# facebookresearch/holo_diffusion

Measured on AMD Instinct MI355X. Metric: denoise-steps/sec + rendered-rays/sec, 64^3x32 grid @400^2 render, higher is better.
Workload: dtype f32

## Files before the change

### holo_diffusion_amd/csrc/holo_knobs.h

```cpp
#pragma once

#include <stdint.h>
#include <stdlib.h>

namespace holo {

#ifdef HOLO_EMU
constexpr bool EMU_BUILD = true;
#else
constexpr bool EMU_BUILD = false;
#endif

constexpr int64_t KNOB_UNSET = INT64_MIN;

#define HOLO_KNOBS(X)                                                                                                      \
  X(num_cus, "HOLO_NUM_CUS", POS, 0, CTX, "planners size grids and split-K for this many CUs (default: the device's)")     \
  X(conv_wino, "HOLO_CONV_WINO", INT, 1, HANDLE, "0: no Winograd copies of the conv weights (forward and dgrad)")          \
  X(conv_wino3, "HOLO_CONV_WINO3", INT, 1, HANDLE_PLAN, "0: no F(2x2x2, 3x3x3) copies / conv_wino3_kernel never chosen")   \
  X(keep_intermediates, "HOLO_KEEP_INTERMEDIATES", CH, '1', HANDLE,                                                        \
    "1: the plan releases no activation, holo_unet_fetch_block works")                                                     \
  X(render_v1, "HOLO_RENDER_V1", SET, 0, HANDLE, "the ray-per-column render kernel for everything")                        \
  X(render2_nw, "HOLO_RENDER2_NW", INT, 0, HANDLE, "8: the 8-wave form of render2_kernel's 12-wave configurations")        \
  X(render2_nrm_nw, "HOLO_RENDER2_NRM_NW", INT, 0, HANDLE,                                                                 \
    "8: rendered normals two waves per SIMD instead of 10 waves (the emulation build always runs 8)")                      \
  X(render_wgs, "HOLO_RENDER_WGS", POS, 0, HANDLE, "persistent render workgroups (default: one per CU)")                   \
  X(render_xcd, "HOLO_RENDER_XCD", RAW, KNOB_UNSET, HANDLE,                                                                \
    "XCD ranges of the render tile order (default 8; 2 in the emulation build; <= 1: plain order)")                        \
  X(render_tail, "HOLO_RENDER_TAIL", RAW, KNOB_UNSET, HANDLE,                                                              \
    "4-ray tiles at the end of every XCD range handed out as single rays (default: about two rounds; 3 in the "            \
    "emulation build; 0: off)")                                                                                            \
  X(render_static_tiles, "HOLO_RENDER_STATIC_TILES", SET, 0, HANDLE, "static tile stride instead of the dynamic hand-out") \
  X(render_timeline, "HOLO_RENDER_TIMELINE", SET, 0, HANDLE, "per-phase clocks of every render launch (synchronises!)")    \
  X(mlp_mean_bwd_chunk, "HOLO_MLP_MEAN_BWD_CHUNK", POS, 0, HANDLE,                                                         \
    "voxels per chunk of holo_mlp_mean_backward (default: what fits 4 GiB of rows; the emulation build: always 2048)")     \
  X(conv_wino_small, "HOLO_CONV_WINO_SMALL", INT, 1, PLAN, "0: under-filled levels take 64-voxel tiles, not Winograd")     \
  X(conv_force_tz2, "HOLO_CONV_FORCE_TZ2", INT, 0, PLAN, "1: 128-voxel tiles (hence the Winograd kernels) on small grids") \
  X(conv_qkv_fused, "HOLO_CONV_QKV_FUSED", INT, 1, PLAN, "0: row-tile qkv convolution + attn_pack_kernel")                 \
  X(conv1x1_bf16_stream, "HOLO_CONV1X1_BF16_STREAM", INT, 1, PLAN, "0: the row-tile kernel for bf16 1x1x1 convolutions")   \
  X(conv1x1_stream_min_m, "HOLO_CONV1X1_STREAM_MIN_M", INT, 131072, PLAN,                                                  \
    "rows from which a raw-input fp32 1x1x1 convolution streams (0: never)")                                               \
  X(conv1x1_small, "HOLO_CONV1X1_SMALL", INT, 1, PLAN, "0: the row-tile kernel for the fp32 attention's 1x1x1 convs")      \
  X(conv_s2t, "HOLO_CONV_S2T", INT, -1, PLAN, "stride-2 bf16 halo kernel: 0 never, 1 wherever defined (default: by fill)") \
  X(conv_bf16t, "HOLO_CONV_BF16T", INT, -1, PLAN, "bf16 wide-tile kernel: 0 never, 1 everywhere (default: by fill / K)")   \
  X(conv_bf16p, "HOLO_CONV_BF16P", INT, -1, PLAN,                                                                          \
    "its persistent form: 0 never, 1 every wide-tile launch, 2 activated input too (default: raw input)")                  \
  X(conv_bf16p_wgs, "HOLO_CONV_BF16P_WGS", INT, 0, PLAN, "at most this many persistent workgroups (0: no cap)")            \
  X(conv_wino3_min_items, "HOLO_CONV_WINO3_MIN_ITEMS", INT, KNOB_UNSET, PLAN,                                              \
    "work items from which conv_wino3_kernel runs (default: num_cus / 2)")                                                 \
  X(conv_wino3_up, "HOLO_CONV_WINO3_UP", INT, 1, PLAN,                                                                     \
    "0: upsampling convolutions on conv_wino3_kernel's generic form (64 pseudo-taps), not its 27-tap form")               \
  X(no_skip_fusion, "HOLO_NO_SKIP_FUSION", SET, 0, PLAN, "a ResBlock's 1x1x1 skip always as its own launch")               \
  X(skip_fusion_below_r, "HOLO_SKIP_FUSION_BELOW_R", RAW, 64, PLAN,                                                        \
    "exact fp32: the skip is fused into the second convolution below this grid edge")                                      \
  X(no_flash_attn, "HOLO_NO_FLASH_ATTN", SET, 0, PLAN, "attention as GEMM + softmax + GEMM")                               \
  X(bf16_flash_min_t, "HOLO_BF16_FLASH_MIN_T", RAW, 1024, PLAN, "tokens from which the bf16 mode takes its bf16 attention") \
  X(flash_split, "HOLO_FLASH_SPLIT", INT, 0, PLAN, "key splits of the fp32 attention, clamped to [1, T/128] (0: by fill)") \
  X(flash_v2_ksplit, "HOLO_FLASH_V2_KSPLIT", INT, 0, PLAN,                                                                 \
    "key splits of the bf16 attention: 1..8 dividing T into multiples of 128, else ignored")                               \
  X(attn_exact, "HOLO_ATTN_EXACT", SET, 0, PLAN, "bf16 attention: the exact loop alone, no LAZY pass")                     \
  X(debug_timestep_load, "HOLO_DEBUG_TIMESTEP_LOAD", INT, 0, PLAN, "how time_embed_kernel loads the timesteps (see it)")   \
  X(dgrad_s2_direct, "HOLO_DGRAD_S2_DIRECT", CH, '1', PLAN, "1: conv_dgrad_s2_kernel for every Downsample dgrad")          \
  X(wgrad_tiles, "HOLO_WGRAD_TILES", POS, 0, PLAN, "> 0: the tile weight-gradient kernel instead of the row-staged one")   \
  X(wgrad_reduce_tile_min, "HOLO_WGRAD_REDUCE_TILE_MIN", RAW, 1024, PLAN,                                                  \
    "64-element tiles from which the weight-gradient reduce runs its tile form")                                           \
  X(debug_plan, "HOLO_DEBUG_PLAN", SET, 0, PLAN, "[plan] lines on stderr: what every convolution / attention launches")    \
  X(viewpool_bwd_v1, "HOLO_VIEWPOOL_BWD_V1", CH, '1', CALL, "1: the register-accumulating view-pool backward kernel")      \
  HOLO_KNOBS_DEV(X)

#ifdef HOLO_DEV_PROBES
#define HOLO_KNOBS_DEV(X)                                                                                                  \
  X(viewpool_bwd_probe, "HOLO_VIEWPOOL_BWD_PROBE", RAW, KNOB_UNSET, CALL,                                                  \
    "view-pool backward: 0 no pass 2, 2 pass 2 without its atomics, 10 + k the atomics of map k alone")                    \
  X(viewpool_bwd_occ, "HOLO_VIEWPOOL_BWD_OCC", CH, '3', CALL, "view-pool backward: 3 = the 166-register build")
#else
#define HOLO_KNOBS_DEV(X)
#endif

typedef int64_t knob_INT_t, knob_RAW_t, knob_POS_t;
typedef bool knob_SET_t, knob_CH_t;
static inline int64_t knob_INT(const char* e, int64_t dflt) { return e && e[0] ? strtoll(e, nullptr, 10) : dflt; }
static inline int64_t knob_RAW(const char* e, int64_t dflt) { return e ? atoll(e) : dflt; }
static inline bool knob_SET(const char* e, int) { return e != nullptr; }
static inline bool knob_CH(const char* e, char c) { return e && e[0] == c; }
static inline int64_t knob_POS(const char* e, int) { return e && atoll(e) > 0 ? atoll(e) : 0; }

struct Knobs {
// ... 14 lines not shown
```

### holo_diffusion_amd/csrc/unet_exec.cpp

```cpp
#include <math.h>
#include <stdarg.h>
#include <stdio.h>
#include <stdlib.h>
#include <string.h>

#include <functional>
#include <map>
#include <optional>
#include <string>
#include <vector>

#include "../../include/holo_abi.h"
#include "conv_weights.h"
#include "holo_common.h"
#include "holo_kernels.h"

namespace holo {

static thread_local char g_err[512] = "";
void set_error(const char* fmt, ...) {
  va_list ap;
  va_start(ap, fmt);
  vsnprintf(g_err, sizeof(g_err), fmt, ap);
  va_end(ap);
}
const char* get_error() { return g_err; }

#define HIP_TRY(expr)                                                                  \
  do {                                                                                 \
    hipError_t _e = (expr);                                                            \
    if (_e != hipSuccess) {                                                            \
      set_error("%s failed: %s (%s:%d)", #expr, hipGetErrorString(_e), __FILE__, __LINE__); \
      return HOLO_E_HIP;                                                               \
    }                                                                                  \
  } while (0)

}

// ... 94 lines not shown
  Act x0, x1, h1, out;
  bool has_x1 = false;
  size_t coefA = 0, coefB = 0, momA = 0, momB = 0;
  const float* film = nullptr;
  size_t qkv = 0, a = 0;
  bool has_skip = false;
};

enum OpKind { OP_IN = 1, OP_TEMB, OP_EMBLIN, OP_STATS, OP_FINAL, OP_CONV, OP_GEMM, OP_SOFTMAX, OP_FLASH, OP_OUT };
struct LayoutIn { float* dst; int C; int64_t V; int dst_bf16; };
struct LayoutOut { const float* src; int C; int64_t V; };
struct TimeEmbed {
  const float *w1, *b1, *w2, *b2;
  float *emb, *emb_silu;
  int load_kind;
};
struct EmbLinears {
  const float *emb_silu, *w, *b;
  float* out;
};
struct GnStats {
  const float* x;
  double* part;
  int C, x_bf16;
  int64_t V;
};
struct GnFinalize {
  const double *part0, *part1;
  int C0, B0, C1, B1;
  int64_t V;
  const float *gamma, *beta, *film;
  int film_stride, film_cout;
  float *coef, *moments;
};
struct Softmax { float* S; int64_t rows; int cols; };
struct Flash {
  AttnParams attn;
  int form;
  float* packed;
  int out_bf16;
  int operands_packed;
  int ksplit, lazy;
};
struct Op {
  OpKind kind;
  union {
    LayoutIn in;
    TimeEmbed temb;
    EmbLinears emblin;
    GnStats stats;
    GnFinalize fin;
    ConvParams conv;
    GemmParams gemm;
    Softmax softmax;
    Flash flash;
    LayoutOut out;
  };
};
static Op make_op(OpKind kind) {
  Op op;
  memset(&op, 0, sizeof op);
  op.kind = kind;
  return op;
}

struct Plan {
  int batch = -1;
  void* ws = nullptr;
  std::vector<Op> ops;
  size_t bytes = 0;
  std::map<std::string, Act> block_outputs;
  int first_conv = -1, last_conv = -1;
  const char* cl_refusal = nullptr;
  bool built_for(int b, const void* w) const { return batch == b && ws == w && !ops.empty(); }
  void invalidate() { *this = Plan(); }
};
struct TrainPlan {
  Plan fwd;
  std::vector<std::function<int(void*)>> bops;
  std::vector<size_t> grad_off;
  size_t gy_off = 0, gx_off = 0;
  size_t bytes = 0;
  bool built_for(int b, const void* w) const { return fwd.built_for(b, w); }
  void invalidate() { *this = TrainPlan(); }
};

}

struct HoloUnet {
  HoloCtx* ctx;
  HoloUnetCfg cfg;
  std::vector<std::vector<Block>> inputs, outputs;
  std::vector<Block> middle;
  int final_ch;
  int ted;
  std::vector<ParamSlot> params;
  std::map<std::string, int> pindex;
  float* pstore = nullptr;
  uint16_t* pstore_bf = nullptr;
  float* pstore_wino = nullptr;
  int compute_mode = 0;
  bool batch_invariant = false;
  int emb_rows = 0;
  std::map<std::string, int> emb_row_off;
  float* emb_w = nullptr;
  float* emb_b = nullptr;
  Knobs knobs;
  Plan plan;
  std::map<std::pair<int, bool>, size_t> ws_cache;
  std::map<std::string, ConvWeights> dgrad;
  std::vector<float*> adam_copies;
  float* dgrad_tmp = nullptr;
  TrainPlan tplan;
  const int64_t* t_dev = nullptr;
  bool tape_valid = false;
  std::map<int, size_t> tws_cache;
};

namespace {

void build_structure(HoloUnet* u) {
  const HoloUnetCfg& c = u->cfg;
  const int mc = c.model_channels;
  int ch = c.channel_mult[0] * mc;
  char buf[128];
  u->inputs.clear();
  u->outputs.clear();
  u->middle.clear();
  u->inputs.push_back({Block{B_CONV, "input_blocks.0.0", c.in_channels, ch}});
  std::vector<int> chans{ch};
  int ds = 1, idx = 1;
  auto has_attn = [&](int d) {
    for (int i = 0; i < c.n_attention_resolutions; ++i)
      if (c.attention_resolutions[i] == d) return true;
    return false;
  };
  for (int level = 0; level < c.n_channel_mult; ++level) {
    const int mult = c.channel_mult[level];
    for (int r = 0; r < c.num_res_blocks; ++r) {
      std::vector<Block> layers;
      snprintf(buf, sizeof buf, "input_blocks.%d.0", idx);
      layers.push_back(Block{B_RES, buf, ch, mult * mc});
      ch = mult * mc;
      if (has_attn(ds)) {
        snprintf(buf, sizeof buf, "input_blocks.%d.1", idx);
        layers.push_back(Block{B_ATTN, buf, ch, ch});
      }
      u->inputs.push_back(layers);
      chans.push_back(ch);
// ... 149 lines not shown
    }
  return n;
}

ConvWeights W(const HoloUnet* u, const std::string& name) {
  auto it = u->pindex.find(name);
  return it == u->pindex.end() ? ConvWeights() : u->params[it->second].w;
}
const float* P(const HoloUnet* u, const std::string& name) { return W(u, name).f32; }

struct ConvDesc {
  const Act* x0 = nullptr;
  const Act* x1 = nullptr;
  int in_R = 0;
  int ups = 0;
  int out_R = 0;
  int stride = 1, ksz = 3;
  ConvWeights w;
  const float* bias = nullptr;
  std::optional<size_t> coef;
  int act = 0;
  const float* residual = nullptr;
  float* out = nullptr;
  int Cout = 0;
  Act* stats_of = nullptr;
  struct {
    const Act* x0 = nullptr;
    const Act* x1 = nullptr;
    ConvWeights w;
    const float* bias = nullptr;
  } skip;
  bool in_f32 = false, out_f32 = false;
  const ConvParams* qkv_pack = nullptr;
  int in_size() const { return in_R ? in_R : x0->R; }
  int out_size() const { return out_R ? out_R : in_size(); }
};

static Act view(size_t off, int C, int R) {
  Act a;
  a.off = off;
  a.C = C;
  a.R = R;
  return a;
}

struct AttnMat {
  float* p;
  int ld;
  int64_t s0, s1;
};
struct AttnDims {
  int N, H, C;
  int64_t T;
  int ch() const { return C / H; }
  float scale2() const {
    const double sc = 1.0 / sqrt(sqrt((double)ch()));
    return (float)(sc * sc);
  }
  AttnMat qkv(float* base, int part) const { return AttnMat{base + part * ch(), 3 * C, T * 3 * C, 3 * ch()}; }
  AttnMat scores(float* S) const { return AttnMat{S, (int)T, (int64_t)H * T * T, T * T}; }
  AttnMat heads(float* a) const { return AttnMat{a, C, T * C, ch()}; }
};
static GemmParams attn_gemm(const AttnDims& d, AttnMat A, AttnMat B, bool b_kmajor, AttnMat C, float alpha) {
  GemmParams g;
  memset(&g, 0, sizeof g);
  g.A = A.p, g.lda = A.ld, g.sa0 = A.s0, g.sa1 = A.s1;
// ... 13 lines not shown
  const HoloUnet* u;
  int N;
  char* base;
  Plan& plan;
  const Knobs knobs = Knobs::from_env();
  std::vector<Op>& ops;
  Arena arena;
  size_t small_top = 0;
  size_t small_cap, arena_base;
  std::vector<Tape>* tape = nullptr;
  size_t last_mom = 0;
  std::string err;
  size_t eml_off = 0, embs_off = 0;
  Act x_in, y_out;

  Planner(const HoloUnet* u_, int N_, void* ws, Plan& plan_) : u(u_), N(N_), base((char*)ws), plan(plan_), ops(plan_.ops) {
    small_cap = Arena::al((size_t)N * 8 * 1024 * 256 * 2 + (size_t)N * (u->emb_rows + 4 * u->ted) * 4 * 2 + 65536);
    arena_base = small_cap;
    arena.keep = u->knobs.keep_intermediates;
  }
  template <class T>
  T* ptr(size_t off) {
    return reinterpret_cast<T*>(base + off);
  }
  int64_t vox(int R) const { return (int64_t)R * R * R; }
  bool bfs() const { return u->compute_mode == 1; }
  int plan_n() const { return u->batch_invariant && !tape ? 1 : N; }

  Act new_act(int C, int R, bool f32 = false) {
    Act a;
    a.C = C;
    a.R = R;
    a.bytes = (size_t)N * vox(R) * C * ((bfs() && !f32) ? 2 : sizeof(float));
    a.off = arena_base + arena.alloc(a.bytes);
    return a;
  }
  void alloc_stats(Act& a, int slabs) {
    a.stats_B = slabs;
    a.stats_bytes = (size_t)N * slabs * a.C * 2 * sizeof(double);
    a.stats_off = arena_base + arena.alloc(a.stats_bytes);
  }
  void release(Act& a) {
    arena.free(a.off - arena_base, a.bytes);
    if (a.stats_bytes) arena.free(a.stats_off - arena_base, a.stats_bytes);
  }
  size_t small_alloc(size_t bytes) {
    size_t off = small_top;
    small_top += Arena::al(bytes);
    return off;
  }
  size_t scratch_alloc(size_t bytes) { return arena_base + arena.alloc(bytes); }
  void scratch_free(size_t off, size_t bytes) { arena.free(off - arena_base, bytes); }

  void emit_stats(Act& a) {
    int B, vpb;
    gn_stats_geometry(a.C, vox(a.R), &B, &vpb);
    alloc_stats(a, B);
    Op op = make_op(OP_STATS);
    op.stats.x = ptr<float>(a.off);
    op.stats.part = ptr<double>(a.stats_off);
    op.stats.C = a.C;
    op.stats.V = vox(a.R);
    op.stats.x_bf16 = bfs() ? 1 : 0;
    ops.push_back(op);
  }
  size_t emit_finalize(const Act& x0, const Act* x1, const std::string& norm, const float* film = nullptr, int film_cout = 0) {
    const int Cin = x0.C + (x1 ? x1->C : 0);
    size_t coef = small_alloc((size_t)N * Cin * 2 * sizeof(float));
    Op op = make_op(OP_FINAL);
    GnFinalize& f = op.fin;
    if (tape) {
      last_mom = small_alloc((size_t)N * Cin * 2 * sizeof(float));
      f.moments = ptr<float>(last_mom);
    }
    f.part0 = ptr<double>(x0.stats_off);
    f.C0 = x0.C;
    f.B0 = x0.stats_B;
    f.part1 = x1 ? ptr<double>(x1->stats_off) : nullptr;
    f.C1 = x1 ? x1->C : 0;
    f.B1 = x1 ? x1->stats_B : 0;
    f.V = vox(x0.R);
    f.gamma = P(u, norm + ".weight");
    f.beta = P(u, norm + ".bias");
    f.film = film;
    f.film_stride = u->emb_rows;
    f.film_cout = film_cout;
    f.coef = ptr<float>(coef);
    ops.push_back(op);
    return coef;
  }
  Tape& record(const Block& b, const Act& x0, const Act& out) {
    tape->emplace_back();
    Tape& t = tape->back();
    t.b = b;
    t.x0 = x0;
    t.out = out;
    return t;
  }
  ConvDesc conv_of(const std::string& layer, const Act& x, const Act& out) {
    ConvDesc d;
    d.x0 = &x;
    d.w = W(u, layer + ".weight");
    d.bias = P(u, layer + ".bias");
    d.out = ptr<float>(out.off);
    d.Cout = out.C;
    return d;
  }
  void hand_over(const ConvWeights& cw, ConvParams& p, bool skip) {
    const bool bf = u->compute_mode != 0, wino = u->compute_mode == 0;
    (skip ? p.skip_w : p.w) = cw.f32;
    (skip ? p.skip_w_bf : p.w_bf) = bf ? cw.bf : nullptr;
    (skip ? p.skip_w_bft : p.w_bft) = bf ? cw.bft : nullptr;
    (skip ? p.skip_w_wino2 : p.w_wino2) = wino ? cw.wino2 : nullptr;
    (skip ? p.skip_w_wino3 : p.w_wino3) = wino ? cw.wino3 : nullptr;
    (skip ? p.skip_CinP : p.CinP) = cw.layout.CinP;
    const ConvWeightLayout& l = cw.layout;
    const int Cin = skip ? p.skip_C0 + p.skip_C1 : p.C0 + p.C1;
    const int tile = conv_cout_tile(p.Cout);
    if (err.empty() && (l.Cout != p.Cout || l.Cin != Cin || (p.Cout + tile - 1) / tile * tile > l.CoutP || l.CoutP != p.CoutP))
      err = "internal: a " + std::to_string(Cin) + " -> " + std::to_string(p.Cout) + " convolution was handed weights packed for " +
            std::to_string(l.Cin) + " -> " + std::to_string(l.Cout) + " (padded to " + std::to_string(l.CinP) + " -> " +
            std::to_string(l.CoutP) + ")";
  }
  void emit_conv(const ConvDesc& d) {
    Op op = make_op(OP_CONV);
    ConvParams& p = op.conv;
    if (const ConvParams* q = d.qkv_pack) {
      p.qkv_q = q->qkv_q, p.qkv_k = q->qkv_k, p.qkv_vt = q->qkv_vt;
      p.qkv_scale = q->qkv_scale, p.qkv_T = q->qkv_T, p.qkv_CH = q->qkv_CH, p.qkv_H = q->qkv_H;
    }
    p.in_bf16 = bfs() && !d.in_f32;
    p.res_bf16 = bfs();
    p.out_bf16 = bfs() && !d.out_f32;
    p.src0 = ptr<float>(d.x0->off);
    p.src1 = d.x1 ? ptr<float>(d.x1->off) : nullptr;
    p.C0 = d.x0->C;
    p.C1 = d.x1 ? d.x1->C : 0;
    p.N = N;
    p.ID = p.IH = p.IW = d.in_size();
    p.ups = d.ups;
    p.OD = p.OH = p.OW = d.out_size();
    p.stride = d.stride;
    p.pad = d.ksz == 3 ? 1 : 0;
    p.ksz = d.ksz;
    p.Cout = d.Cout;
    p.CoutP = d.w.layout.CoutP;
    hand_over(d.w, p, false);
    p.bf16 = u->compute_mode;
    p.coef = d.coef ? ptr<float>(*d.coef) : nullptr;
    p.act = d.act;
    p.bias = d.bias;
    p.residual = d.residual;
    p.out = d.out;
    if (d.skip.w.f32) {
      p.skip_src0 = ptr<float>(d.skip.x0->off);
      p.skip_src1 = d.skip.x1 ? ptr<float>(d.skip.x1->off) : nullptr;
      p.skip_C0 = d.skip.x0->C;
      p.skip_C1 = d.skip.x1 ? d.skip.x1->C : 0;
      hand_over(d.skip.w, p, true);
      p.skip_bias = d.skip.bias;
    }
    ConvParams one = p;
    size_t sb = conv_plan(p, u->ctx->num_cus, knobs, plan_n());
    if (plan_n() != N) {
      one.N = 1;
      conv_plan(one, u->ctx->num_cus, knobs);
      if (err.empty() && (one.kernel != p.kernel || one.tz != p.tz || one.nsplit != p.nsplit ||
                          one.chunks_per_split != p.chunks_per_split || one.skip_chunks_per_split != p.skip_chunks_per_split))
        err = "batch-invariant plan: at batch " + std::to_string(N) + " the " + std::to_string(p.C0 + p.C1) + " -> " +
              std::to_string(p.Cout) + " convolution at " + std::to_string(p.OD) + "^3 cannot keep its batch-1 choice (kernel " +
              std::to_string((int)one.kernel) + ", split-K " + std::to_string(one.nsplit) + " -> kernel " +
              std::to_string((int)p.kernel) + ", split-K " + std::to_string(p.nsplit) + "; an addressing limit of the batch)";
    }
    size_t so = 0;
    if (sb) {
      so = scratch_alloc(sb);
      p.partial = ptr<float>(so);
    }
    const int slabs = d.stats_of ? conv_stats_slabs(p) : 0;
    if (slabs > 0) {
      alloc_stats(*d.stats_of, slabs);
      p.stats = ptr<double>(d.stats_of->stats_off);
    }
    if (sb) scratch_free(so, sb);
    ops.push_back(op);
    if (d.stats_of && slabs == 0) emit_stats(*d.stats_of);
  }

  Act resblock(const Block& b, Act& x0, Act* x1) {
    const std::string& p = b.prefix;
    const int R = x0.R;
    size_t coefA = emit_finalize(x0, x1, p + ".in_layers.0");
    const size_t momA = last_mom;
    Act h1 = new_act(b.cout, R);
    ConvDesc c1 = conv_of(p + ".in_layers.2", x0, h1);
    c1.x1 = x1;
    c1.coef = coefA;
    c1.act = 1;
    c1.stats_of = &h1;
    emit_conv(c1);
    const float* film = ptr<float>(eml_off) + u->emb_row_off.at(p);
    size_t coefB = emit_finalize(h1, nullptr, p + ".out_layers.0", film, b.cout);
    const size_t momB = last_mom;
    const bool has_skip = b.cin != b.cout;
    bool fuse_skip = has_skip && ((R % 8) == 0 || (u->compute_mode == 0 && R < 8)) && b.cout >= 64 && u->compute_mode != 2 &&
                     !knobs.no_skip_fusion;
    if (fuse_skip && u->compute_mode == 0 && R >= knobs.skip_fusion_below_r && (b.cin % 32) == 0 && b.cin <= 256 && (b.cout % 64) == 0)
      fuse_skip = false;
    Act s;
    if (has_skip && !fuse_skip) {
      s = new_act(b.cout, R);
      ConvDesc cs = conv_of(p + ".skip_connection", x0, s);
      cs.x1 = x1;
      cs.ksz = 1;
      emit_conv(cs);
    }
    Act out = new_act(b.cout, R);
    ConvDesc c2 = conv_of(p + ".out_layers.3", h1, out);
    c2.coef = coefB;
    c2.act = 1;
    c2.stats_of = &out;
    if (fuse_skip) {
      c2.skip.x0 = &x0;
      c2.skip.x1 = x1;
      c2.skip.w = W(u, p + ".skip_connection.weight");
      c2.skip.bias = P(u, p + ".skip_connection.bias");
    } else {
      c2.residual = ptr<float>(has_skip ? s.off : x0.off);
    }
    emit_conv(c2);
    release(h1);
    if (has_skip && !fuse_skip) release(s);
    if (tape) {
// ... 149 lines not shown
    embs_off = embs;
    {
      Op op = make_op(OP_TEMB);
      op.temb.w1 = P(u, "time_embed.0.weight");
      op.temb.b1 = P(u, "time_embed.0.bias");
      op.temb.w2 = P(u, "time_embed.2.weight");
      op.temb.b2 = P(u, "time_embed.2.bias");
      op.temb.emb = ptr<float>(emb);
      op.temb.emb_silu = ptr<float>(embs);
      op.temb.load_kind = (int)knobs.debug_timestep_load;
      ops.push_back(op);
    }
    {
      Op op = make_op(OP_EMBLIN);
      op.emblin.emb_silu = ptr<float>(embs);
      op.emblin.w = u->emb_w;
      op.emblin.b = u->emb_b;
      op.emblin.out = ptr<float>(eml_off);
      ops.push_back(op);
    }
    Act x = new_act(c.in_channels, R);
    x_in = x;
    {
      Op op = make_op(OP_IN);
      op.in.dst = ptr<float>(x.off);
      op.in.C = c.in_channels;
      op.in.V = vox(R);
      op.in.dst_bf16 = bfs() ? 1 : 0;
      ops.push_back(op);
    }
    std::vector<Act> hs;
    Act h = x;
    char tag[64];
    for (size_t i = 0; i < u->inputs.size(); ++i) {
      h = run_layers(u->inputs[i], h, nullptr, i == 0);
      hs.push_back(h);
      snprintf(tag, sizeof tag, "input_blocks.%d", (int)i);
      plan.block_outputs[tag] = h;
    }
    h = run_layers(u->middle, h, nullptr, false);
    plan.block_outputs["middle_block"] = h;
    for (size_t i = 0; i < u->outputs.size(); ++i) {
      Act skip = hs.back();
      hs.pop_back();
      h = run_layers(u->outputs[i], h, &skip, true);
      snprintf(tag, sizeof tag, "output_blocks.%d", (int)i);
      plan.block_outputs[tag] = h;
    }
    size_t coef = emit_finalize(h, nullptr, "out.0");
    Act y = new_act(c.out_channels, R, true);
    if (tape) {
      Tape& t = record(Block{B_HEAD, "out", u->final_ch, c.out_channels}, h, y);
      t.coefA = coef;
      t.momA = last_mom;
    }
    ConvDesc head = conv_of("out.2", h, y);
    head.coef = coef;
    head.act = 1;
    head.out_f32 = true;
    emit_conv(head);
    y_out = y;
    release(h);
    {
      Op op = make_op(OP_OUT);
      op.out.src = ptr<float>(y.off);
      op.out.C = c.out_channels;
      op.out.V = vox(R);
      ops.push_back(op);
    }
    release(y);
    if (knobs.debug_plan) {
      int n_fin = 0, n_conv = 0, n_split = 0;
      for (const Op& o : ops) {
        n_fin += o.kind == OP_FINAL;
        if (o.kind != OP_CONV) continue;
        ++n_conv;
        n_split += o.conv.nsplit > 1;
      }
      fprintf(stderr, "[plan] batch %d: %zu ops | %d convs, %d of them split-K (+ a reduce launch) | %d gn_finalize launches\n", N, ops.size(),
              n_conv, n_split, n_fin);
    }
// ... 437 lines not shown
  if (u->plan.built_for(batch, ws)) return 0;
  if (!params_set(u, "holo_unet_forward")) return HOLO_E_STATE;
  if (u->batch_invariant && u->compute_mode != 0) {
    set_error("holo_unet_forward: the batch-invariant plan is exact-fp32 only");
    return HOLO_E_UNSUPPORTED;
  }
  Planner pl(u, batch, ws, u->plan);
  pl.build();
  int rc = 0;
  if (!pl.err.empty()) {
    set_error("holo_unet_forward: %s", pl.err.c_str());
    rc = HOLO_E_UNSUPPORTED;
  } else if (!pl.regions_ok()) {
    set_error("internal: small-buffer regions overflow");
    rc = HOLO_E_INVALID;
  }
  if (rc) u->plan.invalidate();
  return rc;
}

int run_op(const HoloUnet* u, const Op& op, int N, const float* x, const int64_t* t, float* y, void* stream) {
  switch (op.kind) {
    case OP_IN:
      return ncdhw_to_ndhwc_launch(x, op.in.dst, N, op.in.C, op.in.V, 0, stream, op.in.dst_bf16);
    case OP_TEMB:
      return time_embed_launch(t, N, u->cfg.model_channels, u->ted, op.temb.w1, op.temb.b1, op.temb.w2, op.temb.b2,
                               op.temb.emb, op.temb.emb_silu, op.temb.load_kind, stream);
    case OP_EMBLIN:
      return rows_linear_launch(op.emblin.emb_silu, op.emblin.w, op.emblin.b, op.emblin.out, N, u->emb_rows, u->ted, stream);
    case OP_STATS:
      return gn_stats_launch(op.stats.x, op.stats.part, N, op.stats.C, op.stats.V, stream, op.stats.x_bf16);
    case OP_FINAL: {
      const GnFinalize& f = op.fin;
      return gn_finalize_launch(f.part0, f.C0, f.B0, f.part1, f.C1, f.B1, N, f.V, 32, 1e-5f, f.gamma, f.beta, f.film,
                                f.film_stride, f.film_cout, f.coef, stream, f.moments);
    }
    case OP_CONV:
      return conv_launch(op.conv, stream);
    case OP_GEMM:
      return gemm_launch(op.gemm, stream);
    case OP_SOFTMAX:
      return softmax_rows_launch(op.softmax.S, op.softmax.rows, op.softmax.cols, stream);
    case OP_FLASH: {
      const Flash& f = op.flash;
      if (f.form == 2) return flash_attn_bf16v2_launch(f.attn, f.packed, f.out_bf16, f.ksplit, f.lazy, stream, f.operands_packed);
      return flash_attn_launch(f.attn, stream);
    }
    case OP_OUT:
      return ndhwc_to_ncdhw_launch(op.out.src, y, N, op.out.C, op.out.V, stream);
  }
  return 0;
}

int run_plan(const HoloUnet* u, const Plan& plan, const float* x, const int64_t* t, float* y, void* stream) {
  for (const Op& op : plan.ops) {
    if (op.kind == OP_OUT && !y) continue;
    const int rc = run_op(u, op, plan.batch, x, t, y, stream);
    if (rc) return rc < 0 ? rc : HOLO_E_INVALID;
  }
  return 0;
}
int run_backward(const HoloUnet* u, const TrainPlan& tp, const float* grad_out, float* grad_x, void* workspace, void* stream) {
  const HoloUnetCfg& c = u->cfg;
  const int batch = tp.fwd.batch;
  const int64_t V = (int64_t)c.image_size * c.image_size * c.image_size;
  if (ncdhw_to_ndhwc_launch(grad_out, (float*)((char*)workspace + tp.gy_off), batch, c.out_channels, V, 0, stream))
    return HOLO_E_INVALID;
  for (auto& f : tp.bops) {
    const int rc = f(stream);
    if (rc) return rc < 0 ? rc : HOLO_E_INVALID;
  }
  if (grad_x && ndhwc_to_ncdhw_launch((const float*)((char*)workspace + tp.gx_off), grad_x, batch, c.in_channels, V, stream))
    return HOLO_E_INVALID;
  return 0;
}

template <class Launch>
int step_entry(const char* entry, bool args_ok, Launch launch) {
  if (!args_ok) {
    set_error("%s: null/invalid argument", entry);
    return HOLO_E_INVALID;
  }
  return launch() ? HOLO_E_INVALID : 0;
}

}

extern "C" {

int holo_abi_version(void) { return HOLO_ABI_VERSION; }
const char* holo_last_error(void) { return get_error(); }

int holo_ctx_create(int device_id, HoloCtx** out) {
// ... 39 lines not shown
      cfg->image_size % (1 << (cfg->n_channel_mult - 1))) {
    set_error("holo_unet_create: unsupported configuration");
    return HOLO_E_UNSUPPORTED;
  }
  HoloUnet* u = new HoloUnet;
  u->ctx = ctx;
  u->cfg = *cfg;
  build_structure(u);
  enumerate_params(u);
  u->knobs = Knobs::from_env();
  const StoreSizes n = carve_params(u, nullptr, nullptr, nullptr);
  if (hipMalloc((void**)&u->pstore, (size_t)n.f32 * sizeof(float)) != hipSuccess ||
      (n.bf && hipMalloc((void**)&u->pstore_bf, (size_t)n.bf * sizeof(uint16_t)) != hipSuccess) ||
      (n.wino && hipMalloc((void**)&u->pstore_wino, (size_t)n.wino * sizeof(float)) != hipSuccess)) {
    set_error("holo_unet_create: hipMalloc of the parameter stores (%lld floats, %lld bf16 weights, %lld Winograd floats) failed",
              (long long)n.f32, (long long)n.bf, (long long)n.wino);
    holo_unet_destroy(u);
    return HOLO_E_HIP;
  }
  carve_params(u, u->pstore, u->pstore_bf, u->pstore_wino);
  *out = u;
  return 0;
}

int holo_unet_destroy(HoloUnet* net) {
  if (!net) return 0;
  if (net->pstore) (void)hipFree(net->pstore);
  if (net->pstore_bf) (void)hipFree(net->pstore_bf);
  if (net->pstore_wino) (void)hipFree(net->pstore_wino);
  for (auto& kv : net->dgrad)
    for (float* buf : {kv.second.f32, kv.second.wino2, kv.second.wino3})
      if (buf) (void)hipFree(buf);
  if (net->dgrad_tmp) (void)hipFree(net->dgrad_tmp);
  delete net;
  return 0;
}

int holo_unet_num_params(const HoloUnet* net) { return net ? (int)net->params.size() : 0; }

int holo_unet_param_info(const HoloUnet* net, int index, char* name, int name_cap, int64_t shape[8], int* ndim) {
  if (!net || index < 0 || index >= (int)net->params.size()) {
    set_error("holo_unet_param_info: bad index");
    return HOLO_E_INVALID;
  }
  const ParamSlot& s = net->params[index];
  if (name && name_cap > 0) {
    strncpy(name, s.name.c_str(), name_cap - 1);
    name[name_cap - 1] = 0;
  }
  if (ndim) *ndim = (int)s.shape.size();
  if (shape)
    for (size_t i = 0; i < s.shape.size() && i < 8; ++i) shape[i] = s.shape[i];
  return 0;
}

int holo_unet_set_param(HoloUnet* net, const char* name, const void* dev_ptr, int dtype, int ndim,
                        const int64_t* shape, void* stream) {
  if (!net || !name || !dev_ptr) {
    set_error("holo_unet_set_param: null argument");
    return HOLO_E_INVALID;
  }
  if (dtype != HOLO_DTYPE_F32) {
    set_error("holo_unet_set_param: only fp32 parameters are supported");
    return HOLO_E_UNSUPPORTED;
  }
  auto it = net->pindex.find(name);
// ... 67 lines not shown
int holo_unet_forward(HoloUnet* net, int batch, const float* x, const int64_t* timesteps, float* y, void* workspace,
                      size_t workspace_bytes, void* stream) {
  if (!net || !x || !timesteps || !y || !workspace || batch < 1) {
    set_error("holo_unet_forward: null/invalid argument");
    return HOLO_E_INVALID;
  }
  int rc = ensure_plan(net, batch, workspace);
  if (rc) return rc;
  if (workspace_bytes < net->plan.bytes) {
    set_error("holo_unet_forward: workspace too small (%zu < %zu)", workspace_bytes, net->plan.bytes);
    return HOLO_E_WORKSPACE;
  }
  return run_plan(net, net->plan, x, timesteps, y, stream);
}

int holo_unet_forward_cl(HoloUnet* net, int batch, const float* x_cl, const int64_t* timesteps, float* y_cl, void* workspace,
                         size_t workspace_bytes, void* stream) {
  if (!net || !x_cl || !timesteps || !y_cl || !workspace || batch < 1) {
    set_error("holo_unet_forward_cl: null/invalid argument");
    return HOLO_E_INVALID;
  }
  int rc = ensure_plan(net, batch, workspace);
  if (rc) return rc;
  const Plan& plan = net->plan;
  if (workspace_bytes < plan.bytes) {
    set_error("holo_unet_forward_cl: workspace too small (%zu < %zu)", workspace_bytes, plan.bytes);
    return HOLO_E_WORKSPACE;
  }
  if (plan.cl_refusal) {
    set_error("%s", plan.cl_refusal);
    return HOLO_E_UNSUPPORTED;
  }
  const bool bf16_storage = net->compute_mode == 1;
  for (int i = 0; i < (int)plan.ops.size(); ++i) {
    const Op& op = plan.ops[i];
    if (op.kind == OP_IN && bf16_storage) {
      if (f32_to_bf16_launch(x_cl, op.in.dst, (int64_t)batch * op.in.C * op.in.V, stream)) return HOLO_E_INVALID;
      continue;
    }
    if (op.kind == OP_IN || op.kind == OP_OUT) continue;
    if (i == plan.first_conv || i == plan.last_conv) {
      Op o2 = op;
      if (i == plan.first_conv && !bf16_storage) o2.conv.src0 = x_cl;
      if (i == plan.last_conv) o2.conv.out = y_cl;
      rc = run_op(net, o2, batch, x_cl, timesteps, y_cl, stream);
    } else {
      rc = run_op(net, op, batch, x_cl, timesteps, y_cl, stream);
    }
    if (rc) return rc < 0 ? rc : HOLO_E_INVALID;
  }
  return 0;
}

int holo_unet_fetch_block(HoloUnet* net, const char* tag, float* dst, int64_t dst_capacity, int64_t* numel,
                          void* workspace, void* stream) {
  if (!net || !tag || !dst || !workspace) {
    set_error("holo_unet_fetch_block: null argument");
    return HOLO_E_INVALID;
  }
  if (!net->knobs.keep_intermediates) {
    set_error("holo_unet_fetch_block: create the net with HOLO_KEEP_INTERMEDIATES=1");
    return HOLO_E_STATE;
  }
  const Plan& plan = net->plan;
  if (plan.ws != workspace || plan.ops.empty()) {
    set_error("holo_unet_fetch_block: no forward has run on this workspace");
    return HOLO_E_STATE;
  }
  auto it = plan.block_outputs.find(tag);
  if (it == plan.block_outputs.end()) {
    set_error("holo_unet_fetch_block: unknown tag '%s'", tag);
    return HOLO_E_INVALID;
  }
  const Act& a = it->second;
  const int64_t V = (int64_t)a.R * a.R * a.R;
  const int64_t n = (int64_t)plan.batch * V * a.C;
  if (numel) *numel = n;
  if (dst_capacity < n) {
    set_error("holo_unet_fetch_block: destination too small");
    return HOLO_E_INVALID;
  }
  return ndhwc_to_ncdhw_launch((const float*)((char*)workspace + a.off), dst, plan.batch, a.C, V, stream,
                               net->compute_mode == 1 ? 1 : 0);
}
// ... 451 lines not shown
```

Before: 168.4.

## Split up-path concat convolutions and run skip halves on a side stream

For exact fp32 inference, the up-path ResBlock's first convolution over the concatenated [h, skip] input is split into two Winograd launches over weight slices. The skip half, with its own half-GroupNorm finalize, depends only on the stored encoder activation, so it is issued early on a second HIP stream from a fork point at the low-resolution levels. The main-path half later adds it in as a residual after waiting on a join event. This aims to fill idle CUs during the under-occupied low-resolution and middle stages. The cost is extra launches, extra partial buffers held live across the fork, and event synchronisation, with guards against arena allocations overlapping side-lane buffers.

Measured after the change: 170.6 (median of 6 runs). 1.01x the previous value.

```diff
diff --git a/holo_diffusion_amd/csrc/holo_knobs.h b/holo_diffusion_amd/csrc/holo_knobs.h
--- a/holo_diffusion_amd/csrc/holo_knobs.h
+++ b/holo_diffusion_amd/csrc/holo_knobs.h
@@ -52,6 +52,11 @@
   X(no_skip_fusion, "HOLO_NO_SKIP_FUSION", SET, 0, PLAN, "a ResBlock's 1x1x1 skip always as its own launch")               \
   X(skip_fusion_below_r, "HOLO_SKIP_FUSION_BELOW_R", RAW, 64, PLAN,                                                        \
     "exact fp32: the skip is fused into the second convolution below this grid edge")                                      \
+  X(side_lane_cus, "HOLO_SIDE_LANE_CUS", INT, 128, PLAN,                                                                   \
+    "exact fp32 inference: CUs the skip half of a split up-path concat convolution is planned for (0: nothing is split)")  \
+  X(side_lane_min_r, "HOLO_SIDE_LANE_MIN_R", INT, 32, PLAN, "smallest grid edge whose concat convolutions are split")      \
+  X(side_lane_fork_r, "HOLO_SIDE_LANE_FORK_R", INT, 8, PLAN,                                                               \
+    "the side lane starts in front of the first descent level whose grid edge is at most this")                            \
   X(no_flash_attn, "HOLO_NO_FLASH_ATTN", SET, 0, PLAN, "attention as GEMM + softmax + GEMM")                               \
   X(bf16_flash_min_t, "HOLO_BF16_FLASH_MIN_T", RAW, 1024, PLAN, "tokens from which the bf16 mode takes its bf16 attention") \
   X(flash_split, "HOLO_FLASH_SPLIT", INT, 0, PLAN, "key splits of the fp32 attention, clamped to [1, T/128] (0: by fill)") \
diff --git a/holo_diffusion_amd/csrc/unet_exec.cpp b/holo_diffusion_amd/csrc/unet_exec.cpp
--- a/holo_diffusion_amd/csrc/unet_exec.cpp
+++ b/holo_diffusion_amd/csrc/unet_exec.cpp
@@ -4,6 +4,7 @@
 #include <stdlib.h>
 #include <string.h>
 
+#include <algorithm>
 #include <functional>
 #include <map>
 #include <optional>
@@ -164,6 +165,7 @@
   const float *gamma, *beta, *film;
   int film_stride, film_cout;
   float *coef, *moments;
+  int groups;
 };
 struct Softmax { float* S; int64_t rows; int cols; };
 struct Flash {
@@ -188,11 +190,14 @@
     Flash flash;
     LayoutOut out;
   };
+  unsigned char side, fork;
+  short join;
 };
 static Op make_op(OpKind kind) {
   Op op;
   memset(&op, 0, sizeof op);
   op.kind = kind;
+  op.join = -1;
   return op;
 }
 
@@ -204,6 +209,7 @@
   std::map<std::string, Act> block_outputs;
   int first_conv = -1, last_conv = -1;
   const char* cl_refusal = nullptr;
+  int n_joins = 0;
   bool built_for(int b, const void* w) const { return batch == b && ws == w && !ops.empty(); }
   void invalidate() { *this = Plan(); }
 };
@@ -247,6 +253,9 @@
   const int64_t* t_dev = nullptr;
   bool tape_valid = false;
   std::map<int, size_t> tws_cache;
+  void* side_stream = nullptr;
+  void *fork_event = nullptr, *tail_event = nullptr;
+  std::vector<void*> join_events;
 };
 
 namespace {
@@ -462,6 +471,9 @@
   } skip;
   bool in_f32 = false, out_f32 = false;
   const ConvParams* qkv_pack = nullptr;
+  bool w_slice = false;
+  int w_cin0 = 0;
+  int cus = 0;
   int in_size() const { return in_R ? in_R : x0->R; }
   int out_size() const { return out_R ? out_R : in_size(); }
 };
@@ -541,13 +553,13 @@
     a.C = C;
     a.R = R;
     a.bytes = (size_t)N * vox(R) * C * ((bfs() && !f32) ? 2 : sizeof(float));
-    a.off = arena_base + arena.alloc(a.bytes);
+    a.off = guarded(arena_base + arena.alloc(a.bytes), a.bytes);
     return a;
   }
   void alloc_stats(Act& a, int slabs) {
     a.stats_B = slabs;
     a.stats_bytes = (size_t)N * slabs * a.C * 2 * sizeof(double);
-    a.stats_off = arena_base + arena.alloc(a.stats_bytes);
+    a.stats_off = guarded(arena_base + arena.alloc(a.stats_bytes), a.stats_bytes);
   }
   void release(Act& a) {
     arena.free(a.off - arena_base, a.bytes);
@@ -558,7 +570,18 @@
     small_top += Arena::al(bytes);
     return off;
   }
-  size_t scratch_alloc(size_t bytes) { return arena_base + arena.alloc(bytes); }
+  size_t scratch_alloc(size_t bytes) { return guarded(arena_base + arena.alloc(bytes), bytes); }
+  struct SideRange {
+    size_t off, bytes;
+    int join;
+  };
+  std::vector<SideRange> side_live;
+  size_t guarded(size_t off, size_t bytes) {
+    for (const SideRange& r : side_live)
+      if (off < r.off + r.bytes && r.off < off + bytes && err.empty())
+        err = "internal: an allocation between the side lane's fork and join " + std::to_string(r.join) + " overlaps a buffer of that side op";
+    return off;
+  }
   void scratch_free(size_t off, size_t bytes) { arena.free(off - arena_base, bytes); }
 
   void emit_stats(Act& a) {
@@ -595,6 +618,23 @@
     f.film_stride = u->emb_rows;
     f.film_cout = film_cout;
     f.coef = ptr<float>(coef);
+    f.groups = 32;
+    ops.push_back(op);
+    return coef;
+  }
+  size_t emit_finalize_half(const Act& x, int c_first, int cpg, const std::string& norm) {
+    size_t coef = small_alloc((size_t)N * x.C * 2 * sizeof(float));
+    Op op = make_op(OP_FINAL);
+    GnFinalize& f = op.fin;
+    f.part0 = ptr<double>(x.stats_off);
+    f.C0 = x.C;
+    f.B0 = x.stats_B;
+    f.V = vox(x.R);
+    f.gamma = P(u, norm + ".weight") + c_first;
+    f.beta = P(u, norm + ".bias") + c_first;
+    f.film_stride = u->emb_rows;
+    f.coef = ptr<float>(coef);
+    f.groups = x.C / cpg;
     ops.push_back(op);
     return coef;
   }
@@ -615,7 +655,7 @@
     d.Cout = out.C;
     return d;
   }
-  void hand_over(const ConvWeights& cw, ConvParams& p, bool skip) {
+  void hand_over(const ConvWeights& cw, ConvParams& p, bool skip, int cin0 = -1) {
     const bool bf = u->compute_mode != 0, wino = u->compute_mode == 0;
     (skip ? p.skip_w : p.w) = cw.f32;
     (skip ? p.skip_w_bf : p.w_bf) = bf ? cw.bf : nullptr;
@@ -626,14 +666,17 @@
     const ConvWeightLayout& l = cw.layout;
     const int Cin = skip ? p.skip_C0 + p.skip_C1 : p.C0 + p.C1;
     const int tile = conv_cout_tile(p.Cout);
-    if (err.empty() && (l.Cout != p.Cout || l.Cin != Cin || (p.Cout + tile - 1) / tile * tile > l.CoutP || l.CoutP != p.CoutP))
+    const bool slice_ok = cin0 >= 0 && !skip && wino && cw.wino3 && l.taps == 27 && (cin0 % 32) == 0 && (Cin % 32) == 0 && cin0 + Cin <= l.Cin;
+    if (slice_ok) {
+      p.w_wino3 = cw.wino3 + conv_wino3_weight_floats(l.CoutP, cin0, l.taps);
+      p.CinP = Cin;
+    }
+    if (err.empty() && (l.Cout != p.Cout || (l.Cin != Cin && !slice_ok) || (cin0 >= 0 && !slice_ok) || (p.Cout + tile - 1) / tile * tile > l.CoutP || l.CoutP != p.CoutP))
       err = "internal: a " + std::to_string(Cin) + " -> " + std::to_string(p.Cout) + " convolution was handed weights packed for " +
             std::to_string(l.Cin) + " -> " + std::to_string(l.Cout) + " (padded to " + std::to_string(l.CinP) + " -> " +
             std::to_string(l.CoutP) + ")";
   }
-  void emit_conv(const ConvDesc& d) {
-    Op op = make_op(OP_CONV);
-    ConvParams& p = op.conv;
+  size_t plan_conv(const ConvDesc& d, ConvParams& p) {
     if (const ConvParams* q = d.qkv_pack) {
       p.qkv_q = q->qkv_q, p.qkv_k = q->qkv_k, p.qkv_vt = q->qkv_vt;
       p.qkv_scale = q->qkv_scale, p.qkv_T = q->qkv_T, p.qkv_CH = q->qkv_CH, p.qkv_H = q->qkv_H;
@@ -654,7 +697,7 @@
     p.ksz = d.ksz;
     p.Cout = d.Cout;
     p.CoutP = d.w.layout.CoutP;
-    hand_over(d.w, p, false);
+    hand_over(d.w, p, false, d.w_slice ? d.w_cin0 : -1);
     p.bf16 = u->compute_mode;
     p.coef = d.coef ? ptr<float>(*d.coef) : nullptr;
     p.act = d.act;
@@ -670,10 +713,11 @@
       p.skip_bias = d.skip.bias;
     }
     ConvParams one = p;
-    size_t sb = conv_plan(p, u->ctx->num_cus, knobs, plan_n());
+    const int cus = d.cus > 0 ? d.cus : u->ctx->num_cus;
+    size_t sb = conv_plan(p, cus, knobs, plan_n());
     if (plan_n() != N) {
       one.N = 1;
-      conv_plan(one, u->ctx->num_cus, knobs);
+      conv_plan(one, cus, knobs);
       if (err.empty() && (one.kernel != p.kernel || one.tz != p.tz || one.nsplit != p.nsplit ||
                           one.chunks_per_split != p.chunks_per_split || one.skip_chunks_per_split != p.skip_chunks_per_split))
         err = "batch-invariant plan: at batch " + std::to_string(N) + " the " + std::to_string(p.C0 + p.C1) + " -> " +
@@ -681,6 +725,14 @@
               std::to_string((int)one.kernel) + ", split-K " + std::to_string(one.nsplit) + " -> kernel " +
               std::to_string((int)p.kernel) + ", split-K " + std::to_string(p.nsplit) + "; an addressing limit of the batch)";
     }
+    if (d.w_slice && err.empty() && p.kernel != ConvKernel::Wino3)
+      err = "internal: one half of a split concat convolution left conv_wino3_kernel";
+    return sb;
+  }
+  void emit_conv(const ConvDesc& d) {
+    Op op = make_op(OP_CONV);
+    ConvParams& p = op.conv;
+    const size_t sb = plan_conv(d, p);
     size_t so = 0;
     if (sb) {
       so = scratch_alloc(sb);
@@ -696,18 +748,113 @@
     if (d.stats_of && slabs == 0) emit_stats(*d.stats_of);
   }
 
+  struct SidePart {
+    Act P;
+    int id = 0, join = -1;
+    bool consumed = false;
+  };
+  std::map<std::string, SidePart> side_parts;
+  bool side_stream_used() const { return true; }
+  bool split_eligible(const Block& b, const Act& x1, int n_for) {
+    const int C0 = b.cin - x1.C, cpg = b.cin / 32;
+    if (x1.R < knobs.side_lane_min_r || C0 <= 0 || (b.cin % 32) || (C0 % 32) || (C0 % cpg)) return false;
+    const std::string saved = err;
+    const int saved_N = N;
+    N = n_for;
+    const Act x0 = view(x1.off, C0, x1.R), out = view(x1.off, b.cout, x1.R);
+    const std::string layer = b.prefix + ".in_layers.2";
+    bool ok = true;
+    for (int form = 0; form < 3 && ok; ++form) {
+      ConvDesc d = conv_of(layer, form == 2 ? x1 : x0, out);
+      d.x1 = form == 0 ? &x1 : nullptr;
+      d.coef = x1.off;
+      d.act = 1;
+      d.w_slice = form != 0;
+      d.w_cin0 = form == 2 ? C0 : 0;
+      d.cus = form == 2 ? (int)knobs.side_lane_cus : 0;
+      if (form == 1) d.residual = ptr<float>(x1.off);
+      if (form == 2) d.bias = nullptr;
+      ConvParams p;
+      memset(&p, 0, sizeof p);
+      plan_conv(d, p);
+      ok = err.empty() && p.kernel == ConvKernel::Wino3 && !p.wino3_up && (form != 2 || p.nsplit == 1);
+      err = saved;
+    }
+    N = saved_N;
+    return ok;
+  }
+  void plan_side_lane(const std::vector<Act>& hs) {
+    if (tape || u->compute_mode != 0 || knobs.side_lane_cus <= 0) return;
+    if (N > 1 && !u->batch_invariant) return;
+    const size_t fork_at = ops.size(), n_in = u->inputs.size();
+    int n_parts = 0;
+    for (size_t i = 0; i < u->outputs.size(); ++i) {
+      const size_t j = n_in - 1 - i;
+      const Block& b = u->outputs[i][0];
+      if (j >= hs.size() || b.kind != B_RES) continue;
+      const Act& x1 = hs[j];
+      const bool ok = split_eligible(b, x1, N);
+      if (plan_n() != N && ok != split_eligible(b, x1, 1) && err.empty())
+        err = "batch-invariant plan: at batch " + std::to_string(N) + " the concat convolution of " + b.prefix +
+              " cannot be split where the batch-1 plan splits it";
+      if (!ok) continue;
+      const int C0 = b.cin - x1.C, cpg = b.cin / 32;
+      SidePart part;
+      part.id = n_parts++;
+      part.P = new_act(b.cout, x1.R);
+      const size_t coef = emit_finalize_half(x1, C0, cpg, b.prefix + ".in_layers.0");
+      ops.back().side = side_stream_used();
+      ConvDesc d = conv_of(b.prefix + ".in_layers.2", x1, part.P);
+      d.bias = nullptr;
+      d.coef = coef;
+      d.act = 1;
+      d.w_slice = true;
+      d.w_cin0 = C0;
+      d.cus = (int)knobs.side_lane_cus;
+      emit_conv(d);
+      if (ops.back().conv.nsplit != 1 && err.empty()) err = "internal: the skip half of " + b.prefix + " is no direct launch";
+      if (side_stream_used()) {
+        ops.back().side = 1;
+        ops.back().join = (short)(part.join = plan.n_joins++);
+        side_live.push_back({part.P.off, part.P.bytes, part.id});
+        side_live.push_back({x1.off, x1.bytes, part.id});
+        if (x1.stats_bytes) side_live.push_back({x1.stats_off, x1.stats_bytes, part.id});
+      }
+      if (knobs.debug_plan)
+        fprintf(stderr, "[plan] side lane: %s %d + %d -> %d @%d^3 split, skip half on %s, grid_x %d, join %d\n", b.prefix.c_str(), C0, x1.C,
+                b.cout, x1.R, side_stream_used() ? "the side stream" : "the caller's stream", ops.back().conv.grid_x, part.join);
+      side_parts[b.prefix] = part;
+    }
+    if (plan.n_joins) ops[fork_at].fork = 1;
+  }
+
   Act resblock(const Block& b, Act& x0, Act* x1) {
     const std::string& p = b.prefix;
     const int R = x0.R;
-    size_t coefA = emit_finalize(x0, x1, p + ".in_layers.0");
+    const auto sp = x1 ? side_parts.find(p) : side_parts.end();
+    const bool split = sp != side_parts.end();
+    size_t coefA = split ? emit_finalize_half(x0, 0, b.cin / 32, p + ".in_layers.0") : emit_finalize(x0, x1, p + ".in_layers.0");
     const size_t momA = last_mom;
     Act h1 = new_act(b.cout, R);
     ConvDesc c1 = conv_of(p + ".in_layers.2", x0, h1);
-    c1.x1 = x1;
+    c1.x1 = split ? nullptr : x1;
     c1.coef = coefA;
     c1.act = 1;
     c1.stats_of = &h1;
-    emit_conv(c1);
+    if (split) {
+      SidePart& part = sp->second;
+      c1.w_slice = true;
+      c1.residual = ptr<float>(part.P.off);
+      const size_t at = ops.size();
+      emit_conv(c1);
+      ops[at].join = (short)part.join;
+      side_live.erase(std::remove_if(side_live.begin(), side_live.end(), [&](const SideRange& r) { return r.join == part.id; }),
+                      side_live.end());
+      release(part.P);
+      part.consumed = true;
+    } else {
+      emit_conv(c1);
+    }
     const float* film = ptr<float>(eml_off) + u->emb_row_off.at(p);
     size_t coefB = emit_finalize(h1, nullptr, p + ".out_layers.0", film, b.cout);
     const size_t momB = last_mom;
@@ -923,12 +1070,18 @@
     std::vector<Act> hs;
     Act h = x;
     char tag[64];
+    bool forked = false;
     for (size_t i = 0; i < u->inputs.size(); ++i) {
+      if (!forked && (u->inputs[i][0].kind == B_DOWN ? h.R / 2 : h.R) <= knobs.side_lane_fork_r) {
+        plan_side_lane(hs);
+        forked = true;
+      }
       h = run_layers(u->inputs[i], h, nullptr, i == 0);
       hs.push_back(h);
       snprintf(tag, sizeof tag, "input_blocks.%d", (int)i);
       plan.block_outputs[tag] = h;
     }
+    if (!forked) plan_side_lane(hs);
     h = run_layers(u->middle, h, nullptr, false);
     plan.block_outputs["middle_block"] = h;
     for (size_t i = 0; i < u->outputs.size(); ++i) {
@@ -938,6 +1091,8 @@
       snprintf(tag, sizeof tag, "output_blocks.%d", (int)i);
       plan.block_outputs[tag] = h;
     }
+    for (const auto& kv : side_parts)
+      if (!kv.second.consumed && err.empty()) err = "internal: the side part of " + kv.first + " has no consumer";
     size_t coef = emit_finalize(h, nullptr, "out.0");
     Act y = new_act(c.out_channels, R, true);
     if (tape) {
@@ -1441,7 +1596,7 @@
       return gn_stats_launch(op.stats.x, op.stats.part, N, op.stats.C, op.stats.V, stream, op.stats.x_bf16);
     case OP_FINAL: {
       const GnFinalize& f = op.fin;
-      return gn_finalize_launch(f.part0, f.C0, f.B0, f.part1, f.C1, f.B1, N, f.V, 32, 1e-5f, f.gamma, f.beta, f.film,
+      return gn_finalize_launch(f.part0, f.C0, f.B0, f.part1, f.C1, f.B1, N, f.V, f.groups, 1e-5f, f.gamma, f.beta, f.film,
                                 f.film_stride, f.film_cout, f.coef, stream, f.moments);
     }
     case OP_CONV:
@@ -1461,13 +1616,65 @@
   return 0;
 }
 
-int run_plan(const HoloUnet* u, const Plan& plan, const float* x, const int64_t* t, float* y, void* stream) {
-  for (const Op& op : plan.ops) {
-    if (op.kind == OP_OUT && !y) continue;
-    const int rc = run_op(u, op, plan.batch, x, t, y, stream);
-    if (rc) return rc < 0 ? rc : HOLO_E_INVALID;
-  }
+int ensure_lanes(HoloUnet* u, int n_joins) {
+#ifndef HOLO_EMU
+  if (!u->side_stream) HIP_TRY(hipStreamCreateWithFlags((hipStream_t*)&u->side_stream, hipStreamNonBlocking));
+  for (void** e : {&u->fork_event, &u->tail_event})
+    if (!*e) HIP_TRY(hipEventCreateWithFlags((hipEvent_t*)e, hipEventDisableTiming));
+  while ((int)u->join_events.size() < n_joins) {
+    hipEvent_t e;
+    HIP_TRY(hipEventCreateWithFlags(&e, hipEventDisableTiming));
+    u->join_events.push_back(e);
+  }
+#endif
+  (void)u, (void)n_joins;
   return 0;
+}
+
+template <class Run>
+int run_lanes(HoloUnet* u, const Plan& plan, void* stream, Run run) {
+  int rc = 0;
+#ifdef HOLO_EMU
+  for (size_t i = 0; i < plan.ops.size() && !rc; ++i) rc = run((int)i, plan.ops[i], stream);
+#else
+  if (!plan.n_joins) {
+    for (size_t i = 0; i < plan.ops.size() && !rc; ++i) rc = run((int)i, plan.ops[i], stream);
+    return rc ? (rc < 0 ? rc : HOLO_E_INVALID) : 0;
+  }
+  if ((rc = ensure_lanes(u, plan.n_joins))) return rc;
+  const hipStream_t main = (hipStream_t)stream, side = (hipStream_t)u->side_stream;
+  bool forked = false;
+  hipError_t he = hipSuccess;
+  for (size_t i = 0; i < plan.ops.size() && !rc && he == hipSuccess; ++i) {
+    const Op& op = plan.ops[i];
+    if (op.fork) {
+      if ((he = hipEventRecord((hipEvent_t)u->fork_event, main)) != hipSuccess) break;
+      if ((he = hipStreamWaitEvent(side, (hipEvent_t)u->fork_event, 0)) != hipSuccess) break;
+      forked = true;
+    }
+    if (op.side) {
+      rc = run((int)i, op, side);
+      if (!rc && op.join >= 0) he = hipEventRecord((hipEvent_t)u->join_events[op.join], side);
+    } else {
+      if (op.join >= 0 && (he = hipStreamWaitEvent(main, (hipEvent_t)u->join_events[op.join], 0)) != hipSuccess) break;
+      rc = run((int)i, op, main);
+    }
+  }
+  if (he != hipSuccess) {
+    set_error("the side lane of the forward failed: %s", hipGetErrorString(he));
+    rc = HOLO_E_HIP;
+  }
+  if (rc && forked) {
+    if (hipEventRecord((hipEvent_t)u->tail_event, side) == hipSuccess) (void)hipStreamWaitEvent(main, (hipEvent_t)u->tail_event, 0);
+  }
+#endif
+  return rc ? (rc < 0 ? rc : HOLO_E_INVALID) : 0;
+}
+
+int run_plan(HoloUnet* u, const Plan& plan, const float* x, const int64_t* t, float* y, void* stream) {
+  return run_lanes(u, plan, stream, [&](int, const Op& op, void* st) {
+    return op.kind == OP_OUT && !y ? 0 : run_op(u, op, plan.batch, x, t, y, st);
+  });
 }
 int run_backward(const HoloUnet* u, const TrainPlan& tp, const float* grad_out, float* grad_x, void* workspace, void* stream) {
   const HoloUnetCfg& c = u->cfg;
@@ -1573,6 +1780,15 @@
     for (float* buf : {kv.second.f32, kv.second.wino2, kv.second.wino3})
       if (buf) (void)hipFree(buf);
   if (net->dgrad_tmp) (void)hipFree(net->dgrad_tmp);
+#ifndef HOLO_EMU
+  if (net->side_stream) {
+    (void)hipStreamSynchronize((hipStream_t)net->side_stream);
+    (void)hipStreamDestroy((hipStream_t)net->side_stream);
+  }
+  for (void* e : {net->fork_event, net->tail_event})
+    if (e) (void)hipEventDestroy((hipEvent_t)e);
+  for (void* e : net->join_events) (void)hipEventDestroy((hipEvent_t)e);
+#endif
   delete net;
   return 0;
 }
@@ -1706,24 +1922,18 @@
     return HOLO_E_UNSUPPORTED;
   }
   const bool bf16_storage = net->compute_mode == 1;
-  for (int i = 0; i < (int)plan.ops.size(); ++i) {
-    const Op& op = plan.ops[i];
-    if (op.kind == OP_IN && bf16_storage) {
-      if (f32_to_bf16_launch(x_cl, op.in.dst, (int64_t)batch * op.in.C * op.in.V, stream)) return HOLO_E_INVALID;
-      continue;
-    }
-    if (op.kind == OP_IN || op.kind == OP_OUT) continue;
+  return run_lanes(net, plan, stream, [&](int i, const Op& op, void* st) {
+    if (op.kind == OP_IN && bf16_storage)
+      return f32_to_bf16_launch(x_cl, op.in.dst, (int64_t)batch * op.in.C * op.in.V, st) ? (int)HOLO_E_INVALID : 0;
+    if (op.kind == OP_IN || op.kind == OP_OUT) return 0;
     if (i == plan.first_conv || i == plan.last_conv) {
       Op o2 = op;
       if (i == plan.first_conv && !bf16_storage) o2.conv.src0 = x_cl;
       if (i == plan.last_conv) o2.conv.out = y_cl;
-      rc = run_op(net, o2, batch, x_cl, timesteps, y_cl, stream);
-    } else {
-      rc = run_op(net, op, batch, x_cl, timesteps, y_cl, stream);
-    }
-    if (rc) return rc < 0 ? rc : HOLO_E_INVALID;
-  }
-  return 0;
+      return run_op(net, o2, batch, x_cl, timesteps, y_cl, st);
+    }
+    return run_op(net, op, batch, x_cl, timesteps, y_cl, st);
+  });
 }
 
 int holo_unet_fetch_block(HoloUnet* net, const char* tag, float* dst, int64_t dst_capacity, int64_t* numel,
```
